# Infini-AI-Lab/TriForce

Measured on AMD Instinct MI355X. Metric: decode tokens/sec + avg accepted len, Llama-7B-128K @124K ctx, higher is better.
Workload: dtype f16

## Files before the change

### triforce_amd/csrc/attn.hip

```cpp
#include "common.h"
#include "tree_mask.h"

#define NEG_BIG (-1.0e30f)
#define ATTN_SPLIT_BOUNDS __launch_bounds__(256)
constexpr int ATTN_QT2_OCC = 2;
#define COMBINE_GROUPS 8
#define COMBINE_MAX_SPLITS 128
#define FUSED_MERGE_MAX_SPLITS 8
#ifndef FUSED_MERGE_BIG_SPLITS
#define FUSED_MERGE_BIG_SPLITS 64
#endif
#ifndef FUSED_MERGE_BIG_MAX_WGS
#define FUSED_MERGE_BIG_MAX_WGS 256
#endif
#ifndef TF_ATTN_EAGER_TILES
#define TF_ATTN_EAGER_TILES 16
#endif


__device__ __forceinline__ void st_agent(float* p, float v) {
    __hip_atomic_store(p, v, __ATOMIC_RELAXED, __HIP_MEMORY_SCOPE_AGENT);
}
__device__ __forceinline__ float ld_agent(const float* p) {
    return __hip_atomic_load(p, __ATOMIC_RELAXED, __HIP_MEMORY_SCOPE_AGENT);
// ... 1025 lines not shown
                gv[p] = load_half8_stream(vbase + (int64_t)key * stride_t + 8 * lc);
            }
        }
    };
    auto stash = [&](int buf) {
        if constexpr (DMA) return;
        h16* dk = sK + buf * BlkLayout<D>::K_HALFS;
        h16* dv = sVt + buf * BlkLayout<D>::V_HALFS;
#pragma unroll
        for (int p = 0; p < (DMA ? 0 : NPASS); ++p) {
            const int r = p * RPP + lr;
            store_half8(dk + r * RS + 8 * lc, gk[p]);
#pragma unroll
            for (int e = 0; e < 8; ++e)
                dv[(8 * lc + e) * VS + ((((r >> 3) ^ (lc & (SLAB / 8 - 1))) << 3) | (r & 7))] = gv[p][e];
        }
    };

    if (s_begin < s_end) {
        fetch(s_begin, 0);
        stash(0);
    }
    __builtin_amdgcn_s_waitcnt(0x0F70);
    __syncthreads();
    for (int sl = s_begin; sl < s_end; ++sl) {
        const int buf = (sl - s_begin) & 1;
        fetch(min(sl + 1, s_end - 1), buf ^ 1);
        const h16* bk = sK + buf * BlkLayout<D>::K_HALFS;
        const h16* bv = sVt + buf * BlkLayout<D>::V_HALFS;
        bool piped = false;
        if constexpr (TR && !TREE && SLAB == 64) {
            const int last = sl * SLAB + SLAB - 1;
            if (last < sk && last <= sk - sq + qbase) {
                piped = true;
                f32x4 s0a[QT], s0b[QT], s1a[QT], s1b[QT];
#pragma unroll
                for (int qt = 0; qt < QT; ++qt) {
                    s0a[qt] = f32x4{0.f, 0.f, 0.f, 0.f}; s0b[qt] = f32x4{0.f, 0.f, 0.f, 0.f};
                    s1a[qt] = f32x4{0.f, 0.f, 0.f, 0.f}; s1b[qt] = f32x4{0.f, 0.f, 0.f, 0.f};
                }
#pragma unroll
                for (int c = 0; c < NC; ++c) {
                    const int kcol = 8 * ((4 * c + g) ^ li);
                    const half8 ka = load_half8(bk + row_a * RS + kcol);
                    const half8 kb = load_half8(bk + (row_a + 4) * RS + kcol);
#pragma unroll
                    for (int qt = 0; qt < QT; ++qt) {
                        s0a[qt] = __builtin_amdgcn_mfma_f32_16x16x32_f16(ka, st.qf[qt][c], s0a[qt], 0, 0, 0);
                        s0b[qt] = __builtin_amdgcn_mfma_f32_16x16x32_f16(kb, st.qf[qt][c], s0b[qt], 0, 0, 0);
                    }
                }
#pragma unroll
                for (int c = 0; c < NC; ++c) {
                    const int kcol = 8 * ((4 * c + g) ^ li);
                    const half8 ka = load_half8(bk + (32 + row_a) * RS + kcol);
                    const half8 kb = load_half8(bk + (32 + row_a + 4) * RS + kcol);
#pragma unroll
                    for (int qt = 0; qt < QT; ++qt) {
                        s1a[qt] = __builtin_amdgcn_mfma_f32_16x16x32_f16(ka, st.qf[qt][c], s1a[qt], 0, 0, 0);
                        s1b[qt] = __builtin_amdgcn_mfma_f32_16x16x32_f16(kb, st.qf[qt][c], s1b[qt], 0, 0, 0);
                    }
                }
                half8 p0[QT], p1[QT];
                lds_softmax_clear2<D, QT>(st, s0a, s0b, s1a, s1b, scale_log2, p0, p1);
                lds_pv_tr<D, QT>(st, p0, bv, 0, li, g);
                lds_pv_tr<D, QT>(st, p1, bv, 4, li, g);
            }
        }
#pragma unroll
        for (int sub = 0; sub < (piped ? 0 : SLAB / 32); ++sub) {
            const int key0 = sl * SLAB + 32 * sub;
            if (key0 >= sk) break;
            f32x4 sa[QT], sb[QT];
#pragma unroll
            for (int qt = 0; qt < QT; ++qt) {
                sa[qt] = f32x4{0.f, 0.f, 0.f, 0.f};
                sb[qt] = f32x4{0.f, 0.f, 0.f, 0.f};
            }
#pragma unroll
            for (int c = 0; c < NC; ++c) {
                const int kcol = TR ? 8 * ((4 * c + g) ^ li) : 32 * c + 8 * g;
                const half8 ka = load_half8(bk + (32 * sub + row_a) * RS + kcol);
                const half8 kb = load_half8(bk + (32 * sub + row_a + 4) * RS + kcol);
#pragma unroll
                for (int qt = 0; qt < QT; ++qt) {
                    sa[qt] = __builtin_amdgcn_mfma_f32_16x16x32_f16(ka, st.qf[qt][c], sa[qt], 0, 0, 0);
                    sb[qt] = __builtin_amdgcn_mfma_f32_16x16x32_f16(kb, st.qf[qt][c], sb[qt], 0, 0, 0);
                }
            }
            const int last_key = key0 + 31;
            const bool clear = TREE ? (last_key < tm.start && last_key < sk) : (last_key <= sk - sq + qbase);
            if (clear)
                lds_softmax_pv<D, QT, TREE, false>(st, sa, sb, bv, 4 * sub, key0, sk, sq, scale_log2, li, g, qbase, tm);
            else
                lds_softmax_pv<D, QT, TREE, true>(st, sa, sb, bv, 4 * sub, key0, sk, sq, scale_log2, li, g, qbase, tm);
        }
        if (sl + 1 < s_end) stash(buf ^ 1);
        if constexpr (DMA) __builtin_amdgcn_s_waitcnt(0x0F70);
        __syncthreads();
    }

    float* ws_o = ws;
    float* ws_m = ws + (int64_t)H * nsplit * QR * D;
    float* ws_l = ws_m + (int64_t)H * nsplit * QR;
    const int64_t pbase = ((int64_t)h * nsplit + split) * QR;
#pragma unroll
    for (int qt = 0; qt < QT; ++qt) {
        float lsum = st.l[qt];
        lsum += __shfl_xor(lsum, 16, 64);
        lsum += __shfl_xor(lsum, 32, 64);
        const int64_t row = pbase + qbase + qt * 16 + li;
#pragma unroll
        for (int tt = 0; tt < NT; ++tt) *reinterpret_cast<f32x4*>(ws_o + row * D + 16 * tt + 4 * g) = st.acc[qt][tt];
        if (g == 0) {
            ws_m[row] = st.m[qt] * 0.6931471805599453f;
            ws_l[row] = lsum;
        }
    }
}

template <int D, bool TREE>
__global__ __launch_bounds__(256, BLOCK_LDS_OCC) void attn_block_lds_kernel(
    const h16* __restrict__ q, const h16* __restrict__ k, const h16* __restrict__ v, int64_t stride_t,
    int64_t stride_h, int sq, int sk, int H, float scale, int nsplit, float* __restrict__ ws,
    const uint32_t* __restrict__ mask, int mask_words, int mask_row0, int tree_start) {
    const int split = blockIdx.x, h = blockIdx.y;
    const int nslabs = (sk + BLK_SLAB - 1) / BLK_SLAB;
    const int sps = (nslabs + nsplit - 1) / nsplit;
    const int s_begin = split * sps;
    attn_block_lds_body<D, TREE>(q, k, v, stride_t, stride_h, sq, sk, H, scale, nsplit, ws, mask, mask_words, mask_row0,
                                 tree_start, split, h, s_begin, min(nslabs, s_begin + sps));
}

template <int D>
__device__ __forceinline__ void attn_prefill_ahead_body(
    const h16* __restrict__ q, const h16* __restrict__ k, const h16* __restrict__ v, int64_t stride_t,
    int64_t stride_h, int sq, int sk, int H, float scale, int nsplit, float* __restrict__ ws, int split, int h,
    int s_begin, int s_end) {
    static_assert(BlkLayout<D>::TR && BLK_SLAB == 64, "swizzled-K / transpose-read layout, 64-key slabs");
    constexpr int NC = D / 32, NT = D / 16, QT = 2, QR = 128, SLAB = BLK_SLAB, RS = BlkLayout<D>::RS;
    constexpr int VPR = D / 8, RPP = 256 / VPR, NPASS = SLAB / RPP;
    extern __shared__ __attribute__((aligned(16))) unsigned char blk_smem[];
    h16* sK = reinterpret_cast<h16*>(blk_smem);
    h16* sVt = sK + 2 * BlkLayout<D>::K_HALFS;
    const int tid = threadIdx.x, lane = tid & 63, wave = tid >> 6;
    const int li = lane & 15, g = lane >> 4;
    const int qbase = wave * 32;

    AttnState<D, QT> st;
#pragma unroll
    for (int qt = 0; qt < QT; ++qt) {
        const int row = qbase + qt * 16 + li;
#pragma unroll
        for (int c = 0; c < NC; ++c) {
            half8 z = {0, 0, 0, 0, 0, 0, 0, 0};
            st.qf[qt][c] = (row < sq) ? load_half8(q + ((int64_t)row * H + h) * D + 32 * c + 8 * g) : z;
        }
#pragma unroll
        for (int t = 0; t < NT; ++t) st.acc[qt][t] = f32x4{0.f, 0.f, 0.f, 0.f};
        st.m[qt] = NEG_BIG;
        st.l[qt] = 0.f;
    }
    const h16* kbase = k + (int64_t)h * stride_h;
    const h16* vbase = v + (int64_t)h * stride_h;
    const TreeMask tm{nullptr, 0, 0, 0};
    const float scale_log2 = scale * 1.4426950408889634f;
    const int lr = tid / VPR, lc = tid % VPR;
    const int row_a = 8 * (li >> 2) + (li & 3);

    auto dma_slab = [&](const h16* base, h16* dst_buf, int slab, bool is_v) {
#pragma unroll
        for (int p = 0; p < NPASS; ++p) {
            const int r = p * RPP + lr;
            int key = slab * SLAB + r;
            key = key < sk ? key : sk - 1;
            int c;
            if (!is_v) {
                const int fk = (r & 3) | (((r >> 3) & 3) << 2);
                c = lc ^ fk;
            } else {
                const int fv = (r & 3) | (((r >> 3) & 1) << 2);
                c = (((lc >> 1) ^ fv) << 1) | (lc & 1);
            }
            const h16* src = base + (int64_t)key * stride_t + 8 * c;
            h16* dst = dst_buf + (p * RPP + 4 * wave) * D;
            __builtin_amdgcn_global_load_lds((const __attribute__((address_space(1))) void*)src,
                                             (__attribute__((address_space(3))) void*)dst, 16, 0, 0);
        }
    };
    auto fetch_k = [&](int slab, int buf) { dma_slab(kbase, sK + buf * BlkLayout<D>::K_HALFS, slab, false); };
    auto fetch_v = [&](int slab, int buf) { dma_slab(vbase, sVt + buf * BlkLayout<D>::V_HALFS, slab, true); };
    auto qk_slab = [&](const h16* bk, f32x4 (&a0)[QT], f32x4 (&b0)[QT], f32x4 (&a1)[QT], f32x4 (&b1)[QT]) {
#pragma unroll
        for (int qt = 0; qt < QT; ++qt) {
            a0[qt] = f32x4{0.f, 0.f, 0.f, 0.f}; b0[qt] = f32x4{0.f, 0.f, 0.f, 0.f};
            a1[qt] = f32x4{0.f, 0.f, 0.f, 0.f}; b1[qt] = f32x4{0.f, 0.f, 0.f, 0.f};
        }
#pragma unroll
        for (int sub = 0; sub < 2; ++sub)
#pragma unroll
            for (int c = 0; c < NC; ++c) {
                const int kcol = 8 * ((4 * c + g) ^ li);
                const half8 ka = load_half8(bk + (32 * sub + row_a) * RS + kcol);
                const half8 kb = load_half8(bk + (32 * sub + row_a + 4) * RS + kcol);
#pragma unroll
                for (int qt = 0; qt < QT; ++qt) {
                    if (sub == 0) {
                        a0[qt] = __builtin_amdgcn_mfma_f32_16x16x32_f16(ka, st.qf[qt][c], a0[qt], 0, 0, 0);
                        b0[qt] = __builtin_amdgcn_mfma_f32_16x16x32_f16(kb, st.qf[qt][c], b0[qt], 0, 0, 0);
                    } else {
                        a1[qt] = __builtin_amdgcn_mfma_f32_16x16x32_f16(ka, st.qf[qt][c], a1[qt], 0, 0, 0);
                        b1[qt] = __builtin_amdgcn_mfma_f32_16x16x32_f16(kb, st.qf[qt][c], b1[qt], 0, 0, 0);
                    }
                }
            }
    };

    if (s_begin < s_end) {
        f32x4 c0a[QT], c0b[QT], c1a[QT], c1b[QT];
        fetch_k(s_begin, 0);
        fetch_v(s_begin, 0);
        fetch_k(min(s_begin + 1, s_end - 1), 1);
        __builtin_amdgcn_s_waitcnt(0x0F70);
        __syncthreads();
        qk_slab(sK, c0a, c0b, c1a, c1b);
        __syncthreads();
        for (int sl = s_begin; sl < s_end; ++sl) {
            const int i = sl - s_begin;
            fetch_k(min(sl + 2, s_end - 1), i & 1);
            fetch_v(min(sl + 1, s_end - 1), (i + 1) & 1);
            const h16* bk_next = sK + ((i + 1) & 1) * BlkLayout<D>::K_HALFS;
            const h16* bv = sVt + (i & 1) * BlkLayout<D>::V_HALFS;
            f32x4 n0a[QT], n0b[QT], n1a[QT], n1b[QT];
            const int last = sl * SLAB + SLAB - 1;
            if (last < sk && last <= sk - sq + qbase) {
                half8 p0[QT], p1[QT];
                qk_slab(bk_next, n0a, n0b, n1a, n1b);
                lds_softmax_clear2<D, QT>(st, c0a, c0b, c1a, c1b, scale_log2, p0, p1);
                lds_pv_tr<D, QT>(st, p0, bv, 0, li, g);
                lds_pv_tr<D, QT>(st, p1, bv, 4, li, g);
            } else {
                qk_slab(bk_next, n0a, n0b, n1a, n1b);
                const int key0 = sl * SLAB;
                lds_softmax_pv<D, QT, false, true>(st, c0a, c0b, bv, 0, key0, sk, sq, scale_log2, li, g, qbase, tm);
                if (key0 + 32 < sk)
                    lds_softmax_pv<D, QT, false, true>(st, c1a, c1b, bv, 4, key0 + 32, sk, sq, scale_log2, li, g, qbase, tm);
            }
#pragma unroll
            for (int qt = 0; qt < QT; ++qt) {
                c0a[qt] = n0a[qt]; c0b[qt] = n0b[qt]; c1a[qt] = n1a[qt]; c1b[qt] = n1b[qt];
            }
            __builtin_amdgcn_s_waitcnt(0x0F70);
            __syncthreads();
        }
    }

    float* ws_o = ws;
    float* ws_m = ws + (int64_t)H * nsplit * QR * D;
    float* ws_l = ws_m + (int64_t)H * nsplit * QR;
    const int64_t pbase = ((int64_t)h * nsplit + split) * QR;
#pragma unroll
    for (int qt = 0; qt < QT; ++qt) {
        float lsum = st.l[qt];
        lsum += __shfl_xor(lsum, 16, 64);
        lsum += __shfl_xor(lsum, 32, 64);
        const int64_t row = pbase + qbase + qt * 16 + li;
#pragma unroll
        for (int tt = 0; tt < NT; ++tt) *reinterpret_cast<f32x4*>(ws_o + row * D + 16 * tt + 4 * g) = st.acc[qt][tt];
        if (g == 0) {
            ws_m[row] = st.m[qt] * 0.6931471805599453f;
            ws_l[row] = lsum;
        }
    }
}

template <int D>
__global__ __launch_bounds__(256, 2) void attn_prefill_kernel(
    const h16* __restrict__ q, const h16* __restrict__ k, const h16* __restrict__ v, int64_t stride_t,
    int64_t stride_h, int sq, int sk, int H, float scale, int nsplit, float* __restrict__ ws, int nrb, int rbg) {
    const int id = blockIdx.x;
    const int pairs = H * nsplit;
    const int xcd = id & 7, j = id >> 3;
    const int rb_lo = j % rbg, rest = j / rbg;
    const int pair = (rest % (pairs >> 3)) * 8 + xcd;
    const int rb = rb_lo + rbg * (rest / (pairs >> 3));
    if (rb >= nrb) return;
    const int h = pair / nsplit, split = pair - h * nsplit;
    const int r0 = rb * 128;
    const int rows = min(128, sq - r0);
    const int sk_eff = sk - (sq - (r0 + rows));
    const int nslabs_all = (sk + BLK_SLAB - 1) / BLK_SLAB;
    const int nslabs = (sk_eff + BLK_SLAB - 1) / BLK_SLAB;
    const int sps = (nslabs_all + nsplit - 1) / nsplit;
    const int s_begin = split * sps;
    float* ws_rb = ws + (int64_t)rb * H * nsplit * 128 * (D + 2);
    if constexpr (BlkLayout<D>::TR)
        attn_prefill_ahead_body<D>(q + (int64_t)r0 * H * D, k, v, stride_t, stride_h, rows, sk_eff, H, scale, nsplit, ws_rb,
                                   split, h, s_begin, min(nslabs, s_begin + sps));
    else
        attn_block_lds_body<D, false>(q + (int64_t)r0 * H * D, k, v, stride_t, stride_h, rows, sk_eff, H, scale, nsplit, ws_rb,
                                      nullptr, 0, 0, 0, split, h, s_begin, min(nslabs, s_begin + sps));
}

template <int D>
static size_t blk_lds_bytes() {
    return (size_t)2 * (BlkLayout<D>::K_HALFS + BlkLayout<D>::V_HALFS) * sizeof(h16);
}

template <int D>
__global__ __launch_bounds__(D * COMBINE_GROUPS) void attn_combine_kernel(const float* __restrict__ ws,
                                                                          h16* __restrict__ out, int sq, int H,
                                                                          int nsplit, int QR, int64_t osm, int64_t osk) {
    __shared__ float sm_w[COMBINE_MAX_SPLITS];
    __shared__ float sm_l[COMBINE_MAX_SPLITS];
    __shared__ float sm_o[COMBINE_GROUPS][D];
    const int h = blockIdx.x, qq = blockIdx.y, d = threadIdx.x, g = threadIdx.y;
    const int tid = g * D + d;
    const float* ws_o = ws;
    const float* ws_m = ws + (int64_t)H * nsplit * QR * D;
    const float* ws_l = ws_m + (int64_t)H * nsplit * QR;
    const int64_t base = (int64_t)h * nsplit * QR + qq;
    constexpr int CPT = COMBINE_MAX_SPLITS / COMBINE_GROUPS;
    float ov[CPT];
#pragma unroll
    for (int i = 0; i < CPT; ++i) {
        const int sc = min(g + i * COMBINE_GROUPS, nsplit - 1);
        ov[i] = ws_o[(base + (int64_t)sc * QR) * D + d];
    }
    if (tid < nsplit) {
        sm_w[tid] = ws_m[base + (int64_t)tid * QR];
        sm_l[tid] = ws_l[base + (int64_t)tid * QR];
    }
    __syncthreads();
    float mm = NEG_BIG;
    for (int s = 0; s < nsplit; ++s) mm = fmaxf(mm, sm_w[s]);
    __syncthreads();
    if (tid < nsplit) {
        const float w = __expf(sm_w[tid] - mm);
        sm_w[tid] = w;
        sm_l[tid] *= w;
    }
    __syncthreads();
    float o = 0.f;
#pragma unroll
    for (int i = 0; i < CPT; ++i) {
        const int s = g + i * COMBINE_GROUPS;
        if (s < nsplit) o = fmaf(ov[i], sm_w[s], o);
    }
    sm_o[g][d] = o;
    __syncthreads();
    if (g == 0) {
        float l = 0.f;
        for (int s = 0; s < nsplit; ++s) l += sm_l[s];
        float acc = 0.f;
#pragma unroll
        for (int gg = 0; gg < COMBINE_GROUPS; ++gg) acc += sm_o[gg][d];
        out[(int64_t)qq * osm + (int64_t)((h * D + d) >> 3) * osk + (d & 7)] = (h16)(acc / l);
    }
}

template <int D>
__global__ __launch_bounds__(256) void attn_combine_rows_kernel(const float* __restrict__ ws, h16* __restrict__ out,
                                                                int sq, int H, int nsplit, int QR, int block_rows) {
    constexpr int VPL = D / 64;
    static_assert(COMBINE_MAX_SPLITS <= 128, "two weights per lane");
    const int lane = threadIdx.x & 63;
    const int pair = blockIdx.x * 4 + (threadIdx.x >> 6);
    if (pair >= sq * H) return;
    const int row = pair / H, h = pair - row * H;
    const int rb = block_rows > 0 ? row / block_rows : 0;
    const int qq = row - rb * block_rows;
    ws += (int64_t)rb * H * nsplit * QR * (D + 2);
    const float* ws_o = ws;
    const float* ws_m = ws + (int64_t)H * nsplit * QR * D;
    const float* ws_l = ws_m + (int64_t)H * nsplit * QR;
    const int64_t base = (int64_t)h * nsplit * QR + qq;
    const bool has0 = lane < nsplit, has1 = lane + 64 < nsplit;
    const float m0 = has0 ? ws_m[base + (int64_t)lane * QR] : NEG_BIG;
    const float m1 = has1 ? ws_m[base + (int64_t)(lane + 64) * QR] : NEG_BIG;
    const float l0 = has0 ? ws_l[base + (int64_t)lane * QR] : 0.f;
    const float l1 = has1 ? ws_l[base + (int64_t)(lane + 64) * QR] : 0.f;
    const float mm = wave_max(fmaxf(m0, m1));
    const float w0 = has0 ? __expf(m0 - mm) : 0.f;
    const float w1 = has1 ? __expf(m1 - mm) : 0.f;
    const float l = wave_sum(w0 * l0 + w1 * l1);
    float acc[VPL];
#pragma unroll
    for (int e = 0; e < VPL; ++e) acc[e] = 0.f;
    const float* po = ws_o + base * D + lane * VPL;
    const int64_t sstride = (int64_t)QR * D;
    for (int half = 0; half < 2; ++half) {
        const float wreg = half ? w1 : w0;
        const int cnt = min(max(nsplit - 64 * half, 0), 64);
        const float* ph = po + (int64_t)(64 * half) * sstride;
        int s = 0;
        for (; s + 4 <= cnt; s += 4) {
            float v[4][VPL];
#pragma unroll
            for (int j = 0; j < 4; ++j)
#pragma unroll
                for (int e = 0; e < VPL; ++e) v[j][e] = ph[(int64_t)(s + j) * sstride + e];
#pragma unroll
            for (int j = 0; j < 4; ++j) {
                const float w = __shfl(wreg, s + j, 64);
#pragma unroll
                for (int e = 0; e < VPL; ++e) acc[e] = fmaf(v[j][e], w, acc[e]);
            }
        }
        for (; s < cnt; ++s) {
            const float w = __shfl(wreg, s, 64);
#pragma unroll
            for (int e = 0; e < VPL; ++e) acc[e] = fmaf(ph[(int64_t)s * sstride + e], w, acc[e]);
        }
    }
    const float inv = 1.0f / l;
    h16* o = out + (int64_t)pair * D + lane * VPL;
#pragma unroll
    for (int e = 0; e < VPL; ++e) o[e] = (h16)(acc[e] * inv);
}

template <int D>
__global__ __launch_bounds__(256) void attn_rope_on_read_kernel(
    const h16* __restrict__ q, const h16* __restrict__ k, const h16* __restrict__ v, const h16* __restrict__ cosb,
    const h16* __restrict__ sinb, h16* __restrict__ out, int64_t stride_t, int64_t stride_h, int sq, int kv_len,
    int H, float scale) {
    constexpr int NV = D / 8, HV = NV / 2;
    extern __shared__ float smem[];
    const int h = blockIdx.x;
    const int wave = threadIdx.x >> 6, lane = threadIdx.x & 63;
    const int qrow = blockIdx.y * 4 + wave;
    const bool active = qrow < sq;
    float* pw = smem + (size_t)wave * kv_len;
    const int kmax = active ? (kv_len - sq + qrow) : -1;
    float lsum = 0.f;
    if (active) {
        const h16* qp = q + ((int64_t)qrow * H + h) * D;
        half8 qv[NV];
#pragma unroll
        for (int i = 0; i < NV; ++i) qv[i] = load_half8(qp + 8 * i);
        const h16* kb = k + (int64_t)h * stride_h;
        float mloc = NEG_BIG;
        for (int j = lane; j <= kmax; j += 64) {
            const h16* kp = kb + (int64_t)j * stride_t;
            const h16* cp = cosb + (int64_t)j * D;
            const h16* sp = sinb + (int64_t)j * D;
            half8 kv[NV], cv[NV], sv[NV];
#pragma unroll
            for (int i = 0; i < NV; ++i) {
                kv[i] = load_half8(kp + 8 * i);
                cv[i] = load_half8(cp + 8 * i);
                sv[i] = load_half8(sp + 8 * i);
            }
            float s = 0.f;
#pragma unroll
            for (int i = 0; i < HV; ++i)
#pragma unroll
                for (int e = 0; e < 8; ++e) {
                    const h16 x1 = kv[i][e], x2 = kv[i + HV][e];
                    const h16 lo = hadd_rn(hmul_rn(x1, cv[i][e]), hmul_rn((h16)(-(float)x2), sv[i][e]));
                    const h16 hi = hadd_rn(hmul_rn(x2, cv[i + HV][e]), hmul_rn(x1, sv[i + HV][e]));
                    s = fmaf((float)qv[i][e], (float)lo, s);
                    s = fmaf((float)qv[i + HV][e], (float)hi, s);
                }
            s *= scale;
            pw[j] = s;
            mloc = fmaxf(mloc, s);
        }
        const float mx = wave_max(mloc);
        for (int j = lane; j <= kmax; j += 64) {
            const float p = __expf(pw[j] - mx);
            pw[j] = p;
            lsum += p;
        }
        lsum = wave_sum(lsum);
    }
    __syncthreads();
    if (active) {
        const h16* vb = v + (int64_t)h * stride_h;
        for (int d = lane; d < D; d += 64) {
            float o = 0.f;
            for (int j = 0; j <= kmax; ++j) o = fmaf(pw[j], (float)vb[(int64_t)j * stride_t + d], o);
            out[((int64_t)qrow * H + h) * D + d] = (h16)(o / lsum);
        }
    }
}

#define DRAFT_LDS_MAX_KEYS 384
#define DRAFT_KPAD 8
template <int D>
__global__ __launch_bounds__(256) void attn_rope_on_read_mfma_kernel(
    const h16* __restrict__ q, const h16* __restrict__ k, const h16* __restrict__ v, const h16* __restrict__ cosb,
    const h16* __restrict__ sinb, h16* __restrict__ out, int64_t stride_t, int64_t stride_h, int sq, int kv_len,
    int H, float scale) {
    static_assert(D == 64, "draft head_dim");
    constexpr int KS = D + DRAFT_KPAD;
    extern __shared__ __attribute__((aligned(16))) unsigned char smem_raw[];
    const int kvp = (kv_len + 31) & ~31;
    const int PS = kvp + DRAFT_KPAD;
    h16* sK = reinterpret_cast<h16*>(smem_raw);
    h16* sVt = sK + (size_t)kvp * KS;
    h16* sP = sVt + (size_t)D * PS;
    h16* sPl = sP + (size_t)16 * PS;
    float* sS = reinterpret_cast<float*>(sPl + (size_t)16 * PS);
    float* sL = sS + (size_t)16 * kvp;

    const int h = blockIdx.x, q0 = blockIdx.y * 16;
    const int tid = threadIdx.x, lane = tid & 63, wave = tid >> 6;
    const int li = lane & 15, g = lane >> 4;
    const h16* kb = k + (int64_t)h * stride_h;
    const h16* vb = v + (int64_t)h * stride_h;
    const half8 zero8 = {0, 0, 0, 0, 0, 0, 0, 0};

    for (int e = tid; e < kvp * 4; e += 256) {
        const int j = e >> 2, i = e & 3;
        half8 lo = zero8, hi = zero8;
        if (j < kv_len) {
            const h16* kp = kb + (int64_t)j * stride_t;
            const half8 x1 = load_half8(kp + 8 * i), x2 = load_half8(kp + 8 * i + 32);
            const half8 c1 = load_half8(cosb + (int64_t)j * D + 8 * i), c2 = load_half8(cosb + (int64_t)j * D + 8 * i + 32);
            const half8 s1 = load_half8(sinb + (int64_t)j * D + 8 * i), s2 = load_half8(sinb + (int64_t)j * D + 8 * i + 32);
#pragma unroll
            for (int t = 0; t < 8; ++t) {
                lo[t] = hadd_rn(hmul_rn(x1[t], c1[t]), hmul_rn((h16)(-(float)x2[t]), s1[t]));
                hi[t] = hadd_rn(hmul_rn(x2[t], c2[t]), hmul_rn(x1[t], s2[t]));
            }
        }
        store_half8(sK + (size_t)j * KS + 8 * i, lo);
        store_half8(sK + (size_t)j * KS + 8 * i + 32, hi);
    }
    for (int e = tid; e < kvp * 8; e += 256) {
        const int j = e >> 3, i = e & 7;
        const half8 x = (j < kv_len) ? load_half8(vb + (int64_t)j * stride_t + 8 * i) : zero8;
#pragma unroll
        for (int t = 0; t < 8; ++t) sVt[(size_t)(8 * i + t) * PS + j] = x[t];
    }
    half8 qf[D / 32];
    {
        const int row = q0 + li;
#pragma unroll
        for (int c = 0; c < D / 32; ++c)
            qf[c] = (row < sq) ? load_half8(q + ((int64_t)row * H + h) * D + 32 * c + 8 * g) : zero8;
    }
    __syncthreads();

    for (int t = wave; t < kvp / 16; t += 4) {
        f32x4 s = {0.f, 0.f, 0.f, 0.f};
#pragma unroll
        for (int c = 0; c < D / 32; ++c) {
            const half8 bk = load_half8(sK + (size_t)(t * 16 + li) * KS + 32 * c + 8 * g);
            s = __builtin_amdgcn_mfma_f32_16x16x32_f16(qf[c], bk, s, 0, 0, 0);
        }
#pragma unroll
        for (int r = 0; r < 4; ++r) sS[(size_t)(4 * g + r) * kvp + t * 16 + li] = s[r] * scale;
    }
    __syncthreads();

#pragma unroll
    for (int rr = 0; rr < 4; ++rr) {
        const int row = wave * 4 + rr, qrow = q0 + row;
        const int kmax = (qrow < sq) ? (kv_len - sq + qrow) : -1;
        float mloc = NEG_BIG;
        for (int j = lane; j <= kmax; j += 64) mloc = fmaxf(mloc, sS[(size_t)row * kvp + j]);
        const float mx = wave_max(mloc);
        float lsum = 0.f;
        for (int j = lane; j < kvp; j += 64) {
            float p = 0.f;
            if (j <= kmax) {
                p = __expf(sS[(size_t)row * kvp + j] - mx);
                lsum += p;
            }
            const h16 ph = (h16)p;
            sP[(size_t)row * PS + j] = ph;
            sPl[(size_t)row * PS + j] = (h16)(p - (float)ph);
        }
        lsum = wave_sum(lsum);
        if (lane == 0) sL[row] = lsum;
    }
    __syncthreads();

    f32x4 o = {0.f, 0.f, 0.f, 0.f};
    for (int c = 0; c < kvp / 32; ++c) {
        const half8 ap = load_half8(sP + (size_t)li * PS + 32 * c + 8 * g);
        const half8 bv = load_half8(sVt + (size_t)(16 * wave + li) * PS + 32 * c + 8 * g);
        o = __builtin_amdgcn_mfma_f32_16x16x32_f16(ap, bv, o, 0, 0, 0);
        o = __builtin_amdgcn_mfma_f32_16x16x32_f16(load_half8(sPl + (size_t)li * PS + 32 * c + 8 * g), bv, o, 0, 0, 0);
    }
#pragma unroll
    for (int r = 0; r < 4; ++r) {
        const int row = 4 * g + r, qrow = q0 + row;
        if (qrow < sq) out[((int64_t)qrow * H + h) * D + 16 * wave + li] = (h16)(o[r] / sL[row]);
    }
}

static size_t draft_mfma_lds_bytes(int kv_len) {
    const size_t kvp = (size_t)((kv_len + 31) & ~31), PS = kvp + DRAFT_KPAD;
    return kvp * (64 + DRAFT_KPAD) * 2 + 64 * PS * 2 + 2 * 16 * PS * 2 + 16 * kvp * 4 + 16 * 4;
}

extern "C" int64_t tf_attn_decode_ws_floats(int H, int sq, int D, int nsplit) {
    const int QR = ((sq + 15) / 16) * 16;
    return (int64_t)H * nsplit * QR * (D + 2);
}

static int g_attn_rendezvous = 0;
extern "C" int tf_attn_tune(int key, int value) {
    if (key != 0) return -1;
    const int old = g_attn_rendezvous;
    g_attn_rendezvous = value ? 1 : 0;
    return old;
}

extern "C" int tf_attn_decode_pick_nsplit(int H, int sk) {
    const int tiles = (sk + 15) / 16;
    if (H < 1) H = 1;
    int by_grid = 256 / H;
    if (by_grid >= 1 && 256 - by_grid * H >= 16 && 512 / H >= 2 * by_grid && tiles / (512 / H) >= 256) by_grid = 512 / H;
    int by_work = tiles / 8;
    int n = by_work < by_grid ? by_work : by_grid;
    if (n < 1) n = 1;
    if (n > 128) n = 128;
    return n;
}

template <int D, int QT>
static int launch_attn(const void* q, const void* k, const void* v, void* out, int64_t osm, int64_t osk,
                       int64_t stride_t, int64_t stride_h, int sq, int sk, const int32_t* sk_dev, int H, float scale,
                       int nsplit, float* ws, unsigned* tickets, hipStream_t st) {
    dim3 grid(nsplit, H), block(256);
    if (stride_t > 0x7fffffff || stride_h > 0x7fffffff) return TF_EINVAL;
    if (tickets && nsplit > FUSED_MERGE_MAX_SPLITS &&
        (D != 128 || H > 64 || nsplit > FUSED_MERGE_BIG_SPLITS || (int64_t)nsplit * H > FUSED_MERGE_BIG_MAX_WGS ||
         !g_attn_rendezvous))
        tickets = nullptr;
    if constexpr (QT == 2)
        hipLaunchKernelGGL((attn_split_q2_kernel<D>), grid, block, 0, st, (const h16*)q, (const h16*)k, (const h16*)v,
                           sk_dev, sq, sk, H, nsplit, (int)stride_t, (int)stride_h, scale, ws, tickets, (h16*)out, osm, osk);
    else
        hipLaunchKernelGGL((attn_split_kernel<D, QT>), grid, block, 0, st, (const h16*)q, (const h16*)k, (const h16*)v,
                           sk_dev, sq, sk, H, nsplit, (int)stride_t, (int)stride_h, scale, ws, tickets, (h16*)out, osm, osk);
    TF_LAUNCH_CHECK();
    if (tickets) return TF_OK;
    hipLaunchKernelGGL((attn_combine_kernel<D>), dim3(H, sq), dim3(D, COMBINE_GROUPS), 0, st, (const float*)ws,
                       (h16*)out, sq, H, nsplit, QT * 16, osm, osk);
    TF_LAUNCH_CHECK();
    return TF_OK;
}

static int attn_decode_any(const void* q, const void* k, const void* v, void* out, int64_t osm, int64_t osk,
                           int64_t stride_t, int64_t stride_h, int sq, int sk, const int32_t* sk_dev, int H, int D,
                           float scale, int nsplit, float* ws, int64_t ws_floats, unsigned* tickets, void* stream) {
    if (!q || !k || !v || !out || !ws) return TF_EINVAL;
    if (sq < 1 || sq > 32 || sk < 1 || H < 1 || nsplit < 1 || nsplit > COMBINE_MAX_SPLITS) return TF_EINVAL;
    if ((stride_t % 8) || (stride_h % 8)) return TF_EINVAL;
    if (osm < 8 || osk < 8 || (osm % 4) || (osk % 4)) return TF_EINVAL;
    if (ws_floats < tf_attn_decode_ws_floats(H, sq, D, nsplit)) return TF_ENOSPC;
    hipStream_t st = (hipStream_t)stream;
    const int QT = (sq + 15) / 16;
    if (D == 128 && QT == 1) return launch_attn<128, 1>(q, k, v, out, osm, osk, stride_t, stride_h, sq, sk, sk_dev, H, scale, nsplit, ws, tickets, st);
    if (D == 128 && QT == 2) return launch_attn<128, 2>(q, k, v, out, osm, osk, stride_t, stride_h, sq, sk, sk_dev, H, scale, nsplit, ws, tickets, st);
    if (D == 64 && QT == 1) return launch_attn<64, 1>(q, k, v, out, osm, osk, stride_t, stride_h, sq, sk, sk_dev, H, scale, nsplit, ws, tickets, st);
    if (D == 64 && QT == 2) return launch_attn<64, 2>(q, k, v, out, osm, osk, stride_t, stride_h, sq, sk, sk_dev, H, scale, nsplit, ws, tickets, st);
    return TF_EINVAL;
}

extern "C" int tf_attn_decode(const void* q, const void* k, const void* v, void* out, int64_t stride_t,
                              int64_t stride_h, int sq, int sk, const int32_t* sk_dev, int H, int D, float scale,
                              int nsplit, float* ws, int64_t ws_floats, void* stream) {
    return attn_decode_any(q, k, v, out, (int64_t)H * D, 8, stride_t, stride_h, sq, sk, sk_dev, H, D, scale, nsplit, ws,
                           ws_floats, nullptr, stream);
}

extern "C" int tf_attn_decode_fused(const void* q, const void* k, const void* v, void* out, int64_t stride_t,
                                    int64_t stride_h, int sq, int sk, const int32_t* sk_dev, int H, int D, float scale,
                                    int nsplit, float* ws, int64_t ws_floats, uint32_t* tickets, void* stream) {
    if (!tickets) return TF_EINVAL;
    return attn_decode_any(q, k, v, out, (int64_t)H * D, 8, stride_t, stride_h, sq, sk, sk_dev, H, D, scale, nsplit, ws,
                           ws_floats, tickets, stream);
}

extern "C" int tf_attn_decode_act(const void* q, const void* k, const void* v, void* out, int64_t out_sm, int64_t out_sk,
                                  int64_t stride_t, int64_t stride_h, int sq, int sk, const int32_t* sk_dev, int H, int D,
                                  float scale, int nsplit, float* ws, int64_t ws_floats, uint32_t* tickets, void* stream) {
    return attn_decode_any(q, k, v, out, out_sm, out_sk, stride_t, stride_h, sq, sk, sk_dev, H, D, scale, nsplit, ws,
                           ws_floats, tickets, stream);
}

template <int QT>
static int launch_attn_f8(const void* q, const void* k, const void* v, const void* ke, const void* ve, void* out, int64_t osm,
                          int64_t osk, int64_t stride_t, int64_t stride_h, int64_t e_sh, int sq, int sk, const int32_t* sk_dev,
                          int H, float scale, int nsplit, float* ws, unsigned* tickets, hipStream_t st, const void* kt = nullptr,
                          const void* vt = nullptr, int64_t t_st = 0, int64_t t_sh = 0, int skc = 0) {
    constexpr int D = 128;
    if (tickets && nsplit > FUSED_MERGE_MAX_SPLITS &&
        (H > 64 || nsplit > FUSED_MERGE_BIG_SPLITS || (int64_t)nsplit * H > FUSED_MERGE_BIG_MAX_WGS || !g_attn_rendezvous))
        tickets = nullptr;
    if (kt)
        hipLaunchKernelGGL((attn_split_f8_tail_kernel<QT>), dim3(nsplit, H), dim3(256), 0, st, (const h16*)q, (const uint8_t*)k,
                           (const uint8_t*)v, (const h16*)kt, sq, sk, H, nsplit, (int)stride_t, (int)stride_h, scale, ws, tickets,
                           (h16*)out, osm, osk, (const uint8_t*)ke, (const uint8_t*)ve, e_sh, (const h16*)vt, t_st, t_sh, skc);
    else
        hipLaunchKernelGGL((attn_split_f8_kernel<QT>), dim3(nsplit, H), dim3(256), 0, st, (const h16*)q, (const uint8_t*)k,
                           (const uint8_t*)v, sk_dev, sq, sk, H, nsplit, (int)stride_t, (int)stride_h, scale, ws, tickets,
                           (h16*)out, osm, osk, (const uint8_t*)ke, (const uint8_t*)ve, e_sh);
    TF_LAUNCH_CHECK();
    if (tickets) return TF_OK;
    hipLaunchKernelGGL((attn_combine_kernel<D>), dim3(H, sq), dim3(D, COMBINE_GROUPS), 0, st, (const float*)ws,
                       (h16*)out, sq, H, nsplit, QT * 16, osm, osk);
    TF_LAUNCH_CHECK();
    return TF_OK;
}

extern "C" int tf_attn_decode_fp8_act(const void* q, const void* k_codes, const void* v_codes, const void* k_exp,
                                      const void* v_exp, void* out, int64_t out_sm, int64_t out_sk, int64_t stride_t,
                                      int64_t stride_h, int64_t exp_stride_h, int sq, int sk, const int32_t* sk_dev, int H,
                                      int D, float scale, int nsplit, float* ws, int64_t ws_floats, uint32_t* tickets,
                                      void* stream) {
    if (!q || !k_codes || !v_codes || !k_exp || !v_exp || !out || !ws) return TF_EINVAL;
    if (D != 128 || sq < 1 || sq > 32 || sk < 1 || H < 1 || nsplit < 1 || nsplit > COMBINE_MAX_SPLITS) return TF_EINVAL;
    if (stride_t < D || (stride_t % 16) || (stride_h % 16) || stride_t > 0x7fffffff || stride_h > 0x7fffffff) return TF_EINVAL;
    if (exp_stride_h < sk) return TF_EINVAL;
    if (out_sm < 8 || out_sk < 8 || (out_sm % 4) || (out_sk % 4)) return TF_EINVAL;
    if (ws_floats < tf_attn_decode_ws_floats(H, sq, D, nsplit)) return TF_ENOSPC;
    hipStream_t st = (hipStream_t)stream;
    if (sq <= 16)
        return launch_attn_f8<1>(q, k_codes, v_codes, k_exp, v_exp, out, out_sm, out_sk, stride_t, stride_h, exp_stride_h, sq, sk,
                                 sk_dev, H, scale, nsplit, ws, tickets, st);
    return launch_attn_f8<2>(q, k_codes, v_codes, k_exp, v_exp, out, out_sm, out_sk, stride_t, stride_h, exp_stride_h, sq, sk,
                             sk_dev, H, scale, nsplit, ws, tickets, st);
}

extern "C" int tf_attn_decode_fp8_tail_act(const void* q, const void* k_codes, const void* v_codes, const void* k_exp,
                                           const void* v_exp, const void* k_tail, const void* v_tail, void* out, int64_t out_sm,
                                           int64_t out_sk, int64_t stride_t, int64_t stride_h, int64_t exp_stride_h,
                                           int64_t tail_stride_t, int64_t tail_stride_h, int sq, int sk_codes, int n_tail,
                                           const int32_t* sk_dev, int H, int D, float scale, int nsplit, float* ws,
                                           int64_t ws_floats, uint32_t* tickets, void* stream) {
    if (!q || !k_codes || !v_codes || !k_exp || !v_exp || !k_tail || !v_tail || !out || !ws) return TF_EINVAL;
    if (sk_dev) return TF_EINVAL;
    if (D != 128 || sq < 1 || sq > 32 || sk_codes < 1 || n_tail < 1 || n_tail > 32 || sk_codes > 0x7fffffff - 32) return TF_EINVAL;
    if (H < 1 || nsplit < 1 || nsplit > COMBINE_MAX_SPLITS) return TF_EINVAL;
    if (stride_t < D || (stride_t % 16) || (stride_h % 16) || stride_t > 0x7fffffff || stride_h > 0x7fffffff) return TF_EINVAL;
    if (exp_stride_h < sk_codes) return TF_EINVAL;
    if (tail_stride_t < D || (tail_stride_t % 8) || (tail_stride_h % 8)) return TF_EINVAL;
    if (out_sm < 8 || out_sk < 8 || (out_sm % 4) || (out_sk % 4)) return TF_EINVAL;
    if (ws_floats < tf_attn_decode_ws_floats(H, sq, D, nsplit)) return TF_ENOSPC;
    hipStream_t st = (hipStream_t)stream;
    const int sk = sk_codes + n_tail;
    if (sq <= 16)
        return launch_attn_f8<1>(q, k_codes, v_codes, k_exp, v_exp, out, out_sm, out_sk, stride_t, stride_h, exp_stride_h, sq, sk,
                                 nullptr, H, scale, nsplit, ws, tickets, st, k_tail, v_tail, tail_stride_t, tail_stride_h, sk_codes);
    return launch_attn_f8<2>(q, k_codes, v_codes, k_exp, v_exp, out, out_sm, out_sk, stride_t, stride_h, exp_stride_h, sq, sk,
                             nullptr, H, scale, nsplit, ws, tickets, st, k_tail, v_tail, tail_stride_t, tail_stride_h, sk_codes);
}

extern "C" int64_t tf_attn_block_ws_floats(int H, int D, int nsplit) { return (int64_t)H * nsplit * 128 * (D + 2); }

extern "C" int tf_attn_block_pick_nsplit(int H, int sq, int sk) {
    const int tiles = (sk + 15) / 16;
    const int rg = sq <= 32 ? 1 : (sq <= 64 ? 2 : 4);
    int by_work = tiles / (sq <= 32 ? 32 : 16);
    int by_grid = (rg == 4 ? 512 : 1024) / (H > 0 ? H : 1);
    int n = by_work < by_grid ? by_work : by_grid;
    const int cap = COMBINE_MAX_SPLITS / (4 / rg);
    if (n > cap) n = cap;
    if (n < 1) n = 1;
    return n;
}

template <int D, bool TREE>
static int launch_block(const void* q, const void* k, const void* v, void* out, int64_t stride_t, int64_t stride_h,
                        int sq, int sk, int H, float scale, int nsplit, float* ws, const uint32_t* mask,
                        int mask_words, int mask_row0, int tree_start, hipStream_t st) {
    const int rg = sq <= 32 ? 1 : (sq <= 64 ? 2 : 4);
    if (rg == 4) {
        static bool attr_set = false;
        if (!attr_set) {
            hipError_t e = hipFuncSetAttribute((const void*)attn_block_lds_kernel<D, TREE>,
                                               hipFuncAttributeMaxDynamicSharedMemorySize, (int)blk_lds_bytes<D>());
            if (e != hipSuccess) return (int)e;
            attr_set = true;
        }
        hipLaunchKernelGGL((attn_block_lds_kernel<D, TREE>), dim3(nsplit, H), dim3(256), blk_lds_bytes<D>(), st,
                           (const h16*)q, (const h16*)k, (const h16*)v, stride_t, stride_h, sq, sk, H, scale, nsplit, ws,
                           mask, mask_words, mask_row0, tree_start);
    } else
        hipLaunchKernelGGL((attn_block_kernel<D, TREE>), dim3(nsplit, H), dim3(256), 0, st, (const h16*)q,
                           (const h16*)k, (const h16*)v, stride_t, stride_h, sq, sk, H, scale, nsplit, rg, ws, mask,
                           mask_words, mask_row0, tree_start);
    TF_LAUNCH_CHECK();
    if (sq > 32)
        hipLaunchKernelGGL((attn_combine_rows_kernel<D>), dim3((sq * H + 3) / 4), dim3(256), 0, st, (const float*)ws,
                           (h16*)out, sq, H, nsplit * (4 / rg), 32 * rg, 0);
    else
        hipLaunchKernelGGL((attn_combine_kernel<D>), dim3(H, sq), dim3(D, COMBINE_GROUPS), 0, st, (const float*)ws,
                           (h16*)out, sq, H, nsplit * (4 / rg), 32 * rg, (int64_t)H * D, (int64_t)8);
    TF_LAUNCH_CHECK();
    return TF_OK;
}

#define PREFILL_MAX_ROWS 4096
extern "C" int tf_attn_prefill_pick_nsplit(int H, int sq, int sk) {
    const int nrb = (sq + 127) / 128;
    const int slabs = (sk + BLK_SLAB - 1) / BLK_SLAB;
    int n = 1024 / ((H > 0 ? H : 1) * nrb);
    const int by_work = slabs / 16;
    if (n > by_work) n = by_work;
    if (n > COMBINE_MAX_SPLITS) n = COMBINE_MAX_SPLITS;
    if (n < 1) n = 1;
    while ((H * n) % 8) ++n;
    return n;
}

extern "C" int64_t tf_attn_prefill_ws_floats(int H, int sq, int D, int nsplit) {
    return (int64_t)((sq + 127) / 128) * H * nsplit * 128 * (D + 2);
}

template <int D>
static int launch_prefill(const void* q, const void* k, const void* v, void* out, int64_t stride_t, int64_t stride_h,
                          int sq, int sk, int H, float scale, int nsplit, float* ws, hipStream_t st) {
    static bool attr_set = false;
    if (!attr_set) {
        hipError_t e = hipFuncSetAttribute((const void*)attn_prefill_kernel<D>, hipFuncAttributeMaxDynamicSharedMemorySize,
                                           (int)blk_lds_bytes<D>());
        if (e != hipSuccess) return (int)e;
        attr_set = true;
    }
    const int nrb = (sq + 127) / 128, rbg = nrb < 8 ? nrb : 8;
    const int groups = (nrb + rbg - 1) / rbg;
    const int64_t blocks = (int64_t)H * nsplit * rbg * groups;
    hipLaunchKernelGGL((attn_prefill_kernel<D>), dim3((unsigned)blocks), dim3(256), blk_lds_bytes<D>(), st, (const h16*)q,
                       (const h16*)k, (const h16*)v, stride_t, stride_h, sq, sk, H, scale, nsplit, ws, nrb, rbg);
    TF_LAUNCH_CHECK();
    hipLaunchKernelGGL((attn_combine_rows_kernel<D>), dim3((sq * H + 3) / 4), dim3(256), 0, st, (const float*)ws,
                       (h16*)out, sq, H, nsplit, 128, 128);
    TF_LAUNCH_CHECK();
    return TF_OK;
}

extern "C" int tf_attn_prefill(const void* q, const void* k, const void* v, void* out, int64_t stride_t,
                               int64_t stride_h, int sq, int sk, int H, int D, float scale, int nsplit, float* ws,
                               int64_t ws_floats, void* stream) {
    if (!q || !k || !v || !out || !ws) return TF_EINVAL;
    if (sq < 1 || sq > PREFILL_MAX_ROWS || sk < sq || H < 1 || nsplit < 1 || nsplit > COMBINE_MAX_SPLITS) return TF_EINVAL;
    if ((H * nsplit) % 8) return TF_EINVAL;
    if ((stride_t % 8) || (stride_h % 8)) return TF_EINVAL;
    if (ws_floats < tf_attn_prefill_ws_floats(H, sq, D, nsplit)) return TF_ENOSPC;
    hipStream_t st = (hipStream_t)stream;
    if (D == 128) return launch_prefill<128>(q, k, v, out, stride_t, stride_h, sq, sk, H, scale, nsplit, ws, st);
    if (D == 64) return launch_prefill<64>(q, k, v, out, stride_t, stride_h, sq, sk, H, scale, nsplit, ws, st);
    return TF_EINVAL;
}

extern "C" int tf_attn_block(const void* q, const void* k, const void* v, void* out, int64_t stride_t,
                             int64_t stride_h, int sq, int sk, int H, int D, float scale, int nsplit, float* ws,
                             int64_t ws_floats, const uint32_t* mask, int mask_words, int mask_row0, int tree_start,
                             void* stream) {
    if (!q || !k || !v || !out || !ws) return TF_EINVAL;
    if (sq < 1 || sq > 128 || sk < 1 || H < 1 || nsplit < 1) return TF_EINVAL;
    if (!mask && sk < sq) return TF_EINVAL;
    if (mask && (mask_words < 1 || mask_row0 < 0 || tree_start < 0 || tree_start > sk ||
                 sk - tree_start > 32 * mask_words)) return TF_EINVAL;
    const int rg = sq <= 32 ? 1 : (sq <= 64 ? 2 : 4);
    if (nsplit * (4 / rg) > COMBINE_MAX_SPLITS) return TF_EINVAL;
    if ((stride_t % 8) || (stride_h % 8)) return TF_EINVAL;
    if (ws_floats < tf_attn_block_ws_floats(H, D, nsplit)) return TF_ENOSPC;
    hipStream_t st = (hipStream_t)stream;
    if (D == 128)
        return mask ? launch_block<128, true>(q, k, v, out, stride_t, stride_h, sq, sk, H, scale, nsplit, ws, mask,
                                              mask_words, mask_row0, tree_start, st)
                    : launch_block<128, false>(q, k, v, out, stride_t, stride_h, sq, sk, H, scale, nsplit, ws, nullptr,
                                               0, 0, 0, st);
    if (D == 64)
        return mask ? launch_block<64, true>(q, k, v, out, stride_t, stride_h, sq, sk, H, scale, nsplit, ws, mask,
                                             mask_words, mask_row0, tree_start, st)
                    : launch_block<64, false>(q, k, v, out, stride_t, stride_h, sq, sk, H, scale, nsplit, ws, nullptr,
                                              0, 0, 0, st);
    return TF_EINVAL;
}

extern "C" int tf_attn_rope_on_read(const void* q, const void* k, const void* v, const void* cosb, const void* sinb,
                                    void* out, int64_t stride_t, int64_t stride_h, int sq, int kv_len, int H, int D,
                                    float scale, void* stream) {
    if (!q || !k || !v || !cosb || !sinb || !out) return TF_EINVAL;
    if (D != 64 || sq < 1 || kv_len < sq || H < 1) return TF_EINVAL;
    if (kv_len <= DRAFT_LDS_MAX_KEYS) {
        static bool attr_set = false;
        const size_t lds = draft_mfma_lds_bytes(kv_len);
        if (!attr_set) {
            hipError_t e = hipFuncSetAttribute((const void*)attn_rope_on_read_mfma_kernel<64>,
                                               hipFuncAttributeMaxDynamicSharedMemorySize,
                                               (int)draft_mfma_lds_bytes(DRAFT_LDS_MAX_KEYS));
            if (e != hipSuccess) return (int)e;
            attr_set = true;
        }
        dim3 grid(H, (sq + 15) / 16), block(256);
        hipLaunchKernelGGL((attn_rope_on_read_mfma_kernel<64>), grid, block, lds, (hipStream_t)stream, (const h16*)q,
                           (const h16*)k, (const h16*)v, (const h16*)cosb, (const h16*)sinb, (h16*)out, stride_t,
                           stride_h, sq, kv_len, H, scale);
        TF_LAUNCH_CHECK();
        return TF_OK;
    }
    const size_t lds = (size_t)4 * kv_len * sizeof(float);
    if (lds > 64 * 1024) return TF_ERANGE;
    dim3 grid(H, (sq + 3) / 4), block(256);
    hipLaunchKernelGGL((attn_rope_on_read_kernel<64>), grid, block, lds, (hipStream_t)stream, (const h16*)q,
                       (const h16*)k, (const h16*)v, (const h16*)cosb, (const h16*)sinb, (h16*)out, stride_t, stride_h,
                       sq, kv_len, H, scale);
    TF_LAUNCH_CHECK();
    return TF_OK;
}
```

Before: 238.2.

## Add wide 512-thread prefill attention kernel sharing K/V slabs across two row blocks

Adds a prefill attention kernel in which one 512-thread workgroup covers 256 query rows (two 128-row blocks) and both halves share the same LDS-staged K/V slabs, halving K/V global traffic per row. The two wave groups order their QK and softmax/PV work differently and one group runs at raised priority, so MFMA and softmax phases can overlap. When nsplit is 1 the kernel normalizes and writes output directly through LDS, skipping the combine kernel. It is on by default for D=128 through a new tune key. This only affects prefill, so decode throughput is affected only indirectly, and the change adds a larger, more complex kernel with occupancy and correctness risk.

```diff
diff --git a/triforce_amd/csrc/attn.hip b/triforce_amd/csrc/attn.hip
--- a/triforce_amd/csrc/attn.hip
+++ b/triforce_amd/csrc/attn.hip
@@ -1351,6 +1351,239 @@
                                       nullptr, 0, 0, 0, split, h, s_begin, min(nslabs, s_begin + sps));
 }
 
+template <bool V>
+struct BoolTag {
+    static constexpr bool value = V;
+};
+template <int D>
+__device__ __forceinline__ void attn_prefill_wide_body(
+    const h16* __restrict__ q, const h16* __restrict__ k, const h16* __restrict__ v, int64_t stride_t,
+    int64_t stride_h, int sq, int sk, int sk_wg, int H, float scale, int nsplit, float* __restrict__ ws,
+    h16* __restrict__ out, int split, int h, int wave, int s_begin, int s_end, int s_end_wg) {
+    constexpr int KB = 2;
+    static_assert(BlkLayout<D>::TR && BLK_SLAB == 64, "swizzled-K / transpose-read layout, 64-key slabs");
+    constexpr int NC = D / 32, NT = D / 16, QT = 2, QR = 128, SLAB = BLK_SLAB, RS = BlkLayout<D>::RS;
+    constexpr int VPR = D / 8, RPP = 512 / VPR, NPASS = SLAB / RPP;
+    extern __shared__ __attribute__((aligned(16))) unsigned char blk_smem[];
+    h16* sK = reinterpret_cast<h16*>(blk_smem);
+    h16* sVt = sK + KB * BlkLayout<D>::K_HALFS;
+    const int tid = threadIdx.x, lane = tid & 63;
+    const int li = lane & 15, g = lane >> 4;
+    const int qbase = ((tid >> 6) & 3) * 32;
+    const bool live = sq > 0;
+
+    AttnState<D, QT> st;
+#pragma unroll
+    for (int qt = 0; qt < QT; ++qt) {
+        const int row = qbase + qt * 16 + li;
+#pragma unroll
+        for (int c = 0; c < NC; ++c) {
+            half8 z = {0, 0, 0, 0, 0, 0, 0, 0};
+            st.qf[qt][c] = (row < sq) ? load_half8(q + ((int64_t)row * H + h) * D + 32 * c + 8 * g) : z;
+        }
+#pragma unroll
+        for (int t = 0; t < NT; ++t) st.acc[qt][t] = f32x4{0.f, 0.f, 0.f, 0.f};
+        st.m[qt] = NEG_BIG;
+        st.l[qt] = 0.f;
+    }
+    const h16* kbase = k + (int64_t)h * stride_h;
+    const h16* vbase = v + (int64_t)h * stride_h;
+    const TreeMask tm{nullptr, 0, 0, 0};
+    const float scale_log2 = scale * 1.4426950408889634f;
+    const int lr = tid / VPR, lc = tid % VPR;
+    const int row_a = 8 * (li >> 2) + (li & 3);
+
+    auto dma_slab = [&](const h16* base, h16* dst_buf, int slab, bool is_v) {
+#pragma unroll
+        for (int p = 0; p < NPASS; ++p) {
+            const int r = p * RPP + lr;
+            int key = slab * SLAB + r;
+            key = key < sk_wg ? key : sk_wg - 1;
+            int c;
+            if (!is_v) {
+                const int fk = (r & 3) | (((r >> 3) & 3) << 2);
+                c = lc ^ fk;
+            } else {
+                const int fv = (r & 3) | (((r >> 3) & 1) << 2);
+                c = (((lc >> 1) ^ fv) << 1) | (lc & 1);
+            }
+            const h16* src = base + (int64_t)key * stride_t + 8 * c;
+            h16* dst = dst_buf + (p * RPP + 4 * wave) * D;
+            __builtin_amdgcn_global_load_lds((const __attribute__((address_space(1))) void*)src,
+                                             (__attribute__((address_space(3))) void*)dst, 16, 0, 0);
+        }
+    };
+    auto fetch_k = [&](int slab, int buf) { dma_slab(kbase, sK + buf * BlkLayout<D>::K_HALFS, slab, false); };
+    auto fetch_v = [&](int slab, int buf) { dma_slab(vbase, sVt + buf * BlkLayout<D>::V_HALFS, slab, true); };
+    auto qk_slab = [&](const h16* bk, f32x4 (&a0)[QT], f32x4 (&b0)[QT], f32x4 (&a1)[QT], f32x4 (&b1)[QT]) {
+#pragma unroll
+        for (int qt = 0; qt < QT; ++qt) {
+            a0[qt] = f32x4{0.f, 0.f, 0.f, 0.f}; b0[qt] = f32x4{0.f, 0.f, 0.f, 0.f};
+            a1[qt] = f32x4{0.f, 0.f, 0.f, 0.f}; b1[qt] = f32x4{0.f, 0.f, 0.f, 0.f};
+        }
+#pragma unroll
+        for (int sub = 0; sub < 2; ++sub)
+#pragma unroll
+            for (int c = 0; c < NC; ++c) {
+                const int kcol = 8 * ((4 * c + g) ^ li);
+                const half8 ka = load_half8(bk + (32 * sub + row_a) * RS + kcol);
+                const half8 kb = load_half8(bk + (32 * sub + row_a + 4) * RS + kcol);
+#pragma unroll
+                for (int qt = 0; qt < QT; ++qt) {
+                    if (sub == 0) {
+                        a0[qt] = __builtin_amdgcn_mfma_f32_16x16x32_f16(ka, st.qf[qt][c], a0[qt], 0, 0, 0);
+                        b0[qt] = __builtin_amdgcn_mfma_f32_16x16x32_f16(kb, st.qf[qt][c], b0[qt], 0, 0, 0);
+                    } else {
+                        a1[qt] = __builtin_amdgcn_mfma_f32_16x16x32_f16(ka, st.qf[qt][c], a1[qt], 0, 0, 0);
+                        b1[qt] = __builtin_amdgcn_mfma_f32_16x16x32_f16(kb, st.qf[qt][c], b1[qt], 0, 0, 0);
+                    }
+                }
+            }
+    };
+
+    if (s_begin < s_end_wg) {
+        f32x4 c0a[QT], c0b[QT], c1a[QT], c1b[QT];
+        const bool group_b = (wave >> 2) != 0;
+        if (group_b) __builtin_amdgcn_s_setprio(1);
+        fetch_k(s_begin, 0);
+        fetch_v(s_begin, 0);
+        fetch_k(min(s_begin + 1, s_end_wg - 1), 1);
+        __builtin_amdgcn_s_waitcnt(0x0F70);
+        __syncthreads();
+        qk_slab(sK, c0a, c0b, c1a, c1b);
+        __syncthreads();
+        int kslot = 0, sl = s_begin;
+        auto issue = [&]() {
+            const int i = sl - s_begin;
+            fetch_k(min(sl + 2, s_end_wg - 1), kslot);
+            fetch_v(min(sl + 1, s_end_wg - 1), (i + 1) & 1);
+        };
+        auto close = [&]() {
+            kslot = kslot + 1 == KB ? 0 : kslot + 1;
+            __builtin_amdgcn_s_waitcnt(0x0F70);
+            __syncthreads();
+        };
+        auto run = [&](auto tag) {
+            constexpr bool B = decltype(tag)::value;
+            for (; sl < s_end; ++sl) {
+                issue();
+                const int i = sl - s_begin;
+                const h16* bk_next = sK + (kslot + 1 == KB ? 0 : kslot + 1) * BlkLayout<D>::K_HALFS;
+                const h16* bv = sVt + (i & 1) * BlkLayout<D>::V_HALFS;
+                f32x4 n0a[QT], n0b[QT], n1a[QT], n1b[QT];
+                const int last = sl * SLAB + SLAB - 1;
+                if constexpr (!B) qk_slab(bk_next, n0a, n0b, n1a, n1b);
+                if (last < sk && last <= sk - sq + qbase) {
+                    half8 p0[QT], p1[QT];
+                    lds_softmax_clear2<D, QT>(st, c0a, c0b, c1a, c1b, scale_log2, p0, p1);
+                    lds_pv_tr<D, QT>(st, p0, bv, 0, li, g);
+                    lds_pv_tr<D, QT>(st, p1, bv, 4, li, g);
+                } else {
+                    const int key0 = sl * SLAB;
+                    lds_softmax_pv<D, QT, false, true>(st, c0a, c0b, bv, 0, key0, sk, sq, scale_log2, li, g, qbase, tm);
+                    if (key0 + 32 < sk)
+                        lds_softmax_pv<D, QT, false, true>(st, c1a, c1b, bv, 4, key0 + 32, sk, sq, scale_log2, li, g, qbase, tm);
+                }
+                if constexpr (B) qk_slab(bk_next, n0a, n0b, n1a, n1b);
+#pragma unroll
+                for (int qt = 0; qt < QT; ++qt) {
+                    c0a[qt] = n0a[qt]; c0b[qt] = n0b[qt]; c1a[qt] = n1a[qt]; c1b[qt] = n1b[qt];
+                }
+                close();
+            }
+        };
+        if (group_b) run(BoolTag<true>{});
+        else run(BoolTag<false>{});
+        for (; sl < s_end_wg; ++sl) {
+            issue();
+            close();
+        }
+    }
+    if (!live) return;
+
+    if (out) {
+        h16* so = reinterpret_cast<h16*>(blk_smem) + wave * 32 * D;
+#pragma unroll
+        for (int qt = 0; qt < QT; ++qt) {
+            float lsum = st.l[qt];
+            lsum += __shfl_xor(lsum, 16, 64);
+            lsum += __shfl_xor(lsum, 32, 64);
+            const float inv = 1.0f / lsum;
+#pragma unroll
+            for (int tt = 0; tt < NT; ++tt) {
+                float o[4];
+#pragma unroll
+                for (int r = 0; r < 4; ++r) {
+                    o[r] = st.acc[qt][tt][r] * inv;
+                    asm volatile("" : "+v"(o[r]));
+                }
+                const half4 o4 = {(h16)o[0], (h16)o[1], (h16)o[2], (h16)o[3]};
+                const int c = (2 * tt + (g >> 1)) ^ li;
+                *reinterpret_cast<half4*>(so + (qt * 16 + li) * D + 8 * c + 4 * (g & 1)) = o4;
+            }
+        }
+        __builtin_amdgcn_fence(__ATOMIC_RELEASE, "wavefront");
+        __builtin_amdgcn_wave_barrier();
+        __builtin_amdgcn_fence(__ATOMIC_ACQUIRE, "wavefront");
+        const int qb = (wave & 3) * 32;
+#pragma unroll
+        for (int p = 0; p < 8; ++p) {
+            const int r = 4 * p + (lane >> 4), c = lane & 15;
+            const half8 o8 = load_half8(so + r * D + 8 * (c ^ (r & 15)));
+            if (qb + r < sq) store_half8(out + ((int64_t)(qb + r) * H + h) * D + 8 * c, o8);
+        }
+        return;
+    }
+
+    float* ws_o = ws;
+    float* ws_m = ws + (int64_t)H * nsplit * QR * D;
+    float* ws_l = ws_m + (int64_t)H * nsplit * QR;
+    const int64_t pbase = ((int64_t)h * nsplit + split) * QR;
+#pragma unroll
+    for (int qt = 0; qt < QT; ++qt) {
+        float lsum = st.l[qt];
+        lsum += __shfl_xor(lsum, 16, 64);
+        lsum += __shfl_xor(lsum, 32, 64);
+        const int64_t row = pbase + qbase + qt * 16 + li;
+#pragma unroll
+        for (int tt = 0; tt < NT; ++tt) *reinterpret_cast<f32x4*>(ws_o + row * D + 16 * tt + 4 * g) = st.acc[qt][tt];
+        if (g == 0) {
+            ws_m[row] = st.m[qt] * 0.6931471805599453f;
+            ws_l[row] = lsum;
+        }
+    }
+}
+
+template <int D>
+__global__ __launch_bounds__(512, 2) void attn_prefill_wide_kernel(
+    const h16* __restrict__ q, const h16* __restrict__ k, const h16* __restrict__ v, int64_t stride_t,
+    int64_t stride_h, int sq, int sk, int H, float scale, int nsplit, float* __restrict__ ws, int nwb, int wbg,
+    h16* __restrict__ out) {
+    const int id = blockIdx.x;
+    const int pairs = H * nsplit;
+    const int xcd = id & 7, j = id >> 3;
+    const int wb_lo = j % wbg, rest = j / wbg;
+    const int pair = (rest % (pairs >> 3)) * 8 + xcd;
+    const int wb = wb_lo + wbg * (rest / (pairs >> 3));
+    if (wb >= nwb) return;
+    const int h = pair / nsplit, split = pair - h * nsplit;
+    const int wave = __builtin_amdgcn_readfirstlane(threadIdx.x >> 6);
+    const int rb = 2 * wb + (wave >> 2);
+    const int r0 = rb * 128;
+    const int rows = min(128, sq - r0);
+    const int sk_eff = sk - (sq - (r0 + rows));
+    const int sk_wg = sk - (sq - min(sq, 256 * wb + 256));
+    const int nslabs_all = (sk + BLK_SLAB - 1) / BLK_SLAB;
+    const int nslabs = rows > 0 ? (sk_eff + BLK_SLAB - 1) / BLK_SLAB : 0;
+    const int nslabs_wg = (sk_wg + BLK_SLAB - 1) / BLK_SLAB;
+    const int sps = (nslabs_all + nsplit - 1) / nsplit;
+    const int s_begin = split * sps;
+    float* ws_rb = ws + (int64_t)rb * H * nsplit * 128 * (D + 2);
+    attn_prefill_wide_body<D>(q + (int64_t)r0 * H * D, k, v, stride_t, stride_h, rows, sk_eff, sk_wg, H, scale, nsplit, ws_rb,
+                              out ? out + (int64_t)r0 * H * D : nullptr, split, h, wave, s_begin,
+                              min(nslabs, s_begin + sps), min(nslabs_wg, s_begin + sps));
+}
+
 template <int D>
 static size_t blk_lds_bytes() {
     return (size_t)2 * (BlkLayout<D>::K_HALFS + BlkLayout<D>::V_HALFS) * sizeof(h16);
@@ -1652,7 +1885,14 @@
 }
 
 static int g_attn_rendezvous = 0;
+static int g_attn_prefill_form = 1;
 extern "C" int tf_attn_tune(int key, int value) {
+    if (key == 1) {
+        if (value < 0 || value > 1) return -1;
+        const int old = g_attn_prefill_form;
+        g_attn_prefill_form = value;
+        return old;
+    }
     if (key != 0) return -1;
     const int old = g_attn_rendezvous;
     g_attn_rendezvous = value ? 1 : 0;
@@ -1865,6 +2105,8 @@
 }
 
 template <int D>
+static int launch_prefill_merge(void* out, int sq, int H, int nsplit, float* ws, hipStream_t st);
+template <int D>
 static int launch_prefill(const void* q, const void* k, const void* v, void* out, int64_t stride_t, int64_t stride_h,
                           int sq, int sk, int H, float scale, int nsplit, float* ws, hipStream_t st) {
     static bool attr_set = false;
@@ -1880,6 +2122,33 @@
     hipLaunchKernelGGL((attn_prefill_kernel<D>), dim3((unsigned)blocks), dim3(256), blk_lds_bytes<D>(), st, (const h16*)q,
                        (const h16*)k, (const h16*)v, stride_t, stride_h, sq, sk, H, scale, nsplit, ws, nrb, rbg);
     TF_LAUNCH_CHECK();
+    return launch_prefill_merge<D>(out, sq, H, nsplit, ws, st);
+}
+
+template <int D>
+static int launch_prefill_wide(const void* q, const void* k, const void* v, void* out, int64_t stride_t, int64_t stride_h,
+                               int sq, int sk, int H, float scale, int nsplit, float* ws, hipStream_t st) {
+    constexpr int lds = 2 * (BlkLayout<D>::K_HALFS + BlkLayout<D>::V_HALFS) * (int)sizeof(h16);
+    static bool attr_set = false;
+    if (!attr_set) {
+        hipError_t e = hipFuncSetAttribute((const void*)attn_prefill_wide_kernel<D>,
+                                           hipFuncAttributeMaxDynamicSharedMemorySize, lds);
+        if (e != hipSuccess) return (int)e;
+        attr_set = true;
+    }
+    const int nwb = (sq + 255) / 256, wbg = nwb < 8 ? nwb : 8;
+    const int groups = (nwb + wbg - 1) / wbg;
+    const int64_t blocks = (int64_t)H * nsplit * wbg * groups;
+    const bool direct = nsplit == 1;
+    hipLaunchKernelGGL((attn_prefill_wide_kernel<D>), dim3((unsigned)blocks), dim3(512), lds, st, (const h16*)q,
+                       (const h16*)k, (const h16*)v, stride_t, stride_h, sq, sk, H, scale, nsplit, ws, nwb, wbg,
+                       direct ? (h16*)out : (h16*)nullptr);
+    TF_LAUNCH_CHECK();
+    if (direct) return TF_OK;
+    return launch_prefill_merge<D>(out, sq, H, nsplit, ws, st);
+}
+template <int D>
+static int launch_prefill_merge(void* out, int sq, int H, int nsplit, float* ws, hipStream_t st) {
     hipLaunchKernelGGL((attn_combine_rows_kernel<D>), dim3((sq * H + 3) / 4), dim3(256), 0, st, (const float*)ws,
                        (h16*)out, sq, H, nsplit, 128, 128);
     TF_LAUNCH_CHECK();
@@ -1895,6 +2164,8 @@
     if ((stride_t % 8) || (stride_h % 8)) return TF_EINVAL;
     if (ws_floats < tf_attn_prefill_ws_floats(H, sq, D, nsplit)) return TF_ENOSPC;
     hipStream_t st = (hipStream_t)stream;
+    if (D == 128 && g_attn_prefill_form)
+        return launch_prefill_wide<128>(q, k, v, out, stride_t, stride_h, sq, sk, H, scale, nsplit, ws, st);
     if (D == 128) return launch_prefill<128>(q, k, v, out, stride_t, stride_h, sq, sk, H, scale, nsplit, ws, st);
     if (D == 64) return launch_prefill<64>(q, k, v, out, stride_t, stride_h, sq, sk, H, scale, nsplit, ws, st);
     return TF_EINVAL;
```

After: 237.7. No clear change (-0.2%).
